# NeuroDiffGym/neurodiffeq

Hardware: NVIDIA H100
Metric: collocation-points/sec (residual+grad) (higher is better)
Workload: dtype f32

## Files before the change

### neurodiffeq_b200/csrc/pinnjet_common.cuh

```cuda
#pragma once
#include <cuda_runtime.h>
#include <stdint.h>
#include <stdlib.h>
#include "pinnjet_plan.h"

namespace pj {

inline bool pdl_enabled() {
    static const int on = [] {
        const char* e = getenv("PINNJET_PDL");
        return (e && e[0] == '1') ? 1 : 0;
    }();
    return on != 0;
}

template <typename... KArgs, typename... Args>
inline cudaError_t launch_kernel(void (*kern)(KArgs...), dim3 grid, dim3 block, size_t smem, cudaStream_t s, bool dependent,
                                 Args&&... args) {
    cudaLaunchConfig_t cfg = {};
    cfg.gridDim = grid;
    cfg.blockDim = block;
    cfg.dynamicSmemBytes = smem;
    cfg.stream = s;
    cudaLaunchAttribute attr[1];
// ... 201 lines not shown

template <int S = 1, typename R>
__device__ __forceinline__ R pg_reduce_scatter8(const R (&v)[8], int pg_lane) {
    const bool b2 = pg_lane & 4, b1 = pg_lane & 2, b0 = pg_lane & 1;
    R w[4], x[2];
#pragma unroll
    for (int i = 0; i < 4; ++i)
        w[i] = (b2 ? v[i + 4] : v[i]) + __shfl_xor_sync(0xffffffffu, b2 ? v[i] : v[i + 4], 4 * S);
#pragma unroll
    for (int i = 0; i < 2; ++i)
        x[i] = (b1 ? w[i + 2] : w[i]) + __shfl_xor_sync(0xffffffffu, b1 ? w[i] : w[i + 2], 2 * S);
    return (b0 ? x[1] : x[0]) + __shfl_xor_sync(0xffffffffu, b0 ? x[0] : x[1], S);
}
template <int S = 1, typename R>
__device__ __forceinline__ R pg_reduce_scatter4(const R (&v)[4], int pg_lane) {
    const bool b2 = pg_lane & 4, b1 = pg_lane & 2;
    R w[2];
#pragma unroll
    for (int i = 0; i < 2; ++i)
        w[i] = (b2 ? v[i + 2] : v[i]) + __shfl_xor_sync(0xffffffffu, b2 ? v[i] : v[i + 2], 4 * S);
    R x = (b1 ? w[1] : w[0]) + __shfl_xor_sync(0xffffffffu, b1 ? w[0] : w[1], 2 * S);
    return x + __shfl_xor_sync(0xffffffffu, x, S);
}

__device__ __forceinline__ float tanh_fast(float x) {
    const float ax = fabsf(x), t = x * x;
    float p = fmaf(-0.006276387721300125f, t, 0.021116213873028755f);
    p = fmaf(p, t, -0.053875137120485306f);
    p = fmaf(p, t, 0.13332924246788025f);
    p = fmaf(p, t, -0.3333333134651184f);
    const float small = fmaf(x * t, p, x);
    float e;
    asm("ex2.approx.ftz.f32 %0, %1;" : "=f"(e) : "f"(fminf(ax, 15.0f) * 2.885390081777927f));
    float r;
    asm("rcp.approx.ftz.f32 %0, %1;" : "=f"(r) : "f"(e + 1.0f));
    const float big = copysignf(fmaf(-2.0f, r, 1.0f), x);
    return ax < 0.6f ? small : big;
}

__device__ __forceinline__ void act_d2(int act, float z0, float& a0, float& s1, float& s2) {
    if (act == PJ_ACT_TANH) {
        a0 = tanh_fast(z0);
        s1 = fmaf(-a0, a0, 1.0f);
        s2 = -2.0f * a0 * s1;
    } else {
        sincosf(z0, &a0, &s1);
// ... 276 lines not shown
#pragma unroll
        for (int q = 0; q < Q; ++q) b[q] = bn[q];
    }
}

__device__ __forceinline__ void split_tf32(float x, uint32_t& big, uint32_t& small) {
    big = (__float_as_uint(x) + 0x1000u) & 0xffffe000u;
    small = __float_as_uint(x - __uint_as_float(big));
}
__device__ __forceinline__ void mma_tf32(float (&d)[4], const uint32_t (&a)[4], const uint32_t (&b)[2]) {
    asm volatile("mma.sync.aligned.m16n8k8.row.col.f32.tf32.tf32.f32 {%0,%1,%2,%3}, {%4,%5,%6,%7}, {%8,%9}, {%0,%1,%2,%3};"
                 : "+f"(d[0]), "+f"(d[1]), "+f"(d[2]), "+f"(d[3])
                 : "r"(a[0]), "r"(a[1]), "r"(a[2]), "r"(a[3]), "r"(b[0]), "r"(b[1]));
}
__device__ __forceinline__ void mma_tf32x3(float (&d)[4], const uint32_t (&ab)[4], const uint32_t (&as)[4], const uint32_t (&bb)[2],
                                           const uint32_t (&bs)[2]) {
    mma_tf32(d, as, bb);
    mma_tf32(d, ab, bs);
    mma_tf32(d, ab, bb);
}

template <typename R, int NTC, int C, int N3>
constexpr bool mma_gemms() { return sizeof(R) == 4 && N3 == 0 && NTC == 128 && C <= 6; }

template <int P, int C, bool AHEAD = true>
__device__ __forceinline__ void gemm_rows_mma(float (&acc)[4][C][P], const float* __restrict__ a_ptr, int RS, int T,
                                              const float* __restrict__ b_ptr, int ldb, int nrows, int lane) {
    static_assert(P == 2 || P == 4, "float2 / float4 point rows");
    const int g = lane >> 2, t = lane & 3;
    const float* ap = a_ptr + 2 * t * RS;
    const float* bp = b_ptr - 4 * t + 4 * (g >> 1) + (g & 1) + 2 * t * ldb;
    struct Ops {
        float a[2][C][P], b[2][2];
    };
    auto load = [&](int k0, Ops& o) {
#pragma unroll
        for (int i = 0; i < 2; ++i) {
            const float* ar = ap + (k0 + i) * RS;
#pragma unroll
            for (int c = 0; c < C; ++c) {
                if constexpr (P == 4) {
                    const float4 v = *reinterpret_cast<const float4*>(ar + c * T);
                    o.a[i][c][0] = v.x;
                    o.a[i][c][1] = v.y;
                    o.a[i][c][2] = v.z;
                    o.a[i][c][3] = v.w;
                } else {
                    const float2 v = *reinterpret_cast<const float2*>(ar + c * T);
                    o.a[i][c][0] = v.x;
                    o.a[i][c][1] = v.y;
                }
            }
#pragma unroll
            for (int ni = 0; ni < 2; ++ni) o.b[ni][i] = bp[(k0 + i) * ldb + 2 * ni];
        }
    };
    if (nrows <= 0) return;
    float d[C][P / 2][2][4];
#pragma unroll
    for (int c = 0; c < C; ++c)
#pragma unroll
        for (int h = 0; h < P / 2; ++h)
#pragma unroll
            for (int ni = 0; ni < 2; ++ni)
#pragma unroll
                for (int e = 0; e < 4; ++e) d[c][h][ni][e] = acc[2 * ni + (e & 1)][c][2 * h + (e >> 1)];
    Ops cur;
    if constexpr (AHEAD) load(0, cur);
#pragma unroll 1
    for (int k0 = 0; k0 < nrows; k0 += 8) {
        Ops nxt;
        if constexpr (AHEAD) load(min(k0 + 8, nrows - 8), nxt);
        else load(k0, cur);
        uint32_t bb[2][2], bs[2][2];
#pragma unroll
        for (int ni = 0; ni < 2; ++ni)
#pragma unroll
            for (int i = 0; i < 2; ++i) split_tf32(cur.b[ni][i], bb[ni][i], bs[ni][i]);
#pragma unroll
        for (int c = 0; c < C; ++c)
#pragma unroll
            for (int h = 0; h < P / 2; ++h) {
                uint32_t ab[4], as[4];
                split_tf32(cur.a[0][c][2 * h], ab[0], as[0]);
                split_tf32(cur.a[0][c][2 * h + 1], ab[1], as[1]);
                split_tf32(cur.a[1][c][2 * h], ab[2], as[2]);
                split_tf32(cur.a[1][c][2 * h + 1], ab[3], as[3]);
#pragma unroll
                for (int ni = 0; ni < 2; ++ni) mma_tf32x3(d[c][h][ni], ab, as, bb[ni], bs[ni]);
            }
        if constexpr (AHEAD) cur = nxt;
    }
#pragma unroll
    for (int c = 0; c < C; ++c)
#pragma unroll
        for (int h = 0; h < P / 2; ++h)
#pragma unroll
            for (int ni = 0; ni < 2; ++ni)
#pragma unroll
                for (int e = 0; e < 4; ++e) acc[2 * ni + (e & 1)][c][2 * h + (e >> 1)] = d[c][h][ni][e];
}

template <typename R, int P, bool SCALAR>
struct GemmAcc {
    typedef typename Pair<R>::type elem;
    static constexpr int n = P / 2;
};
template <int P>
struct GemmAcc<float, P, true> {
    typedef float elem;
    static constexpr int n = P;
};

template <int P, typename PairT>
__device__ __forceinline__ auto pick(const PairT (&v)[P / 2], int p) {
    const auto t = unpack2(v[p >> 1]);
    return (p & 1) ? t.y : t.x;
}
template <int P>
__device__ __forceinline__ float pick(const float (&v)[P], int p) { return v[p]; }

// ... 33 lines not shown
```

### neurodiffeq_b200/csrc/pinnjet_inst.cu

```cuda
#ifndef PJ_WL
#define PJ_WL 0
#endif
#ifndef PJ_N3
#define PJ_N3 0
#endif
#ifndef PJ_XACT
#define PJ_XACT 0
#endif
#define PJ_TC_UNIT (!PJ_F64 && PJ_N3 == 0 && !PJ_XACT)

#include "pinnjet_k1.cuh"
#include "pinnjet_k2.cuh"
#if PJ_TC_UNIT
#include "pinnjet_k1tc3.cuh"
#include "pinnjet_k2tc2.cuh"
#endif

#define PJ_CAT4(a, b, c, d) a##b##_##c##_##d
#define PJ_CAT5(a, b, c, d, e) a##b##_##c##_##d##_##e
#define PJ_NAME4(prefix, n1, n2, wl) PJ_CAT4(prefix, n1, n2, wl)
#define PJ_NAME5(prefix, n1, n2, wl, n3) PJ_CAT5(prefix, n1, n2, wl, n3)
#if PJ_N3 > 0
#define PJ_NAME(prefix, n1, n2) PJ_NAME5(prefix, n1, n2, PJ_WL, PJ_N3)
#else
// ... 39 lines not shown
    const long long i = (long long)blockIdx.x * RED_PARAMS + il;
    red[g][il] = i < n_theta ? red_group_sum(gpart, n_parts, n_theta, i, g) : 0.0f;
    __syncthreads();
    if (g == 0 && i < n_theta) grad[i] += red_combine(red, il);
}

template <typename R>
static cudaError_t launch_reduce_t(const R* gpart, int n_parts, long long n_theta, R* grad, cudaStream_t s) {
    return launch_kernel(k2_reduce_kernel<R>, dim3((unsigned)((n_theta + RED_PARAMS - 1) / RED_PARAMS)), dim3(RED_PARAMS * RED_GROUPS), 0, s,
                         true, gpart, n_parts, n_theta, grad);
}
cudaError_t launch_reduce(const float* gpart, int n_parts, long long n_theta, float* grad, cudaStream_t s) {
    return launch_reduce_t(gpart, n_parts, n_theta, grad, s);
}
cudaError_t launch_reduce_f64(const double* gpart, int n_parts, long long n_theta, double* grad, cudaStream_t s) {
    return launch_reduce_t(gpart, n_parts, n_theta, grad, s);
}

#else

#if PJ_F64
typedef K1ArgsF64 K1A;
typedef K2ArgsF64 K2A;
constexpr int kEsz = 8;
constexpr int kMinB1_128 = 1, kMinB2_128 = 1;
#else
typedef K1Args K1A;
typedef K2Args K2A;
constexpr int kEsz = 4;
constexpr int kMinB1_128 = 3, kMinB2_128 = 2;
#endif
constexpr int kP = ffma_tile_points(1 + PJ_N1 + PJ_N2 + PJ_N3, kEsz);

template <typename Args>
struct Variant {
    void (*kern)(Args);
    int threads;
    cudaError_t ready;
};
template <typename Args>
static Variant<Args> variant(void (*kern)(Args), int threads) {
    return {kern, threads, cudaFuncSetAttribute(kern, cudaFuncAttributeMaxDynamicSharedMemorySize, SMEM_LIMIT)};
}

static Variant<K1A> k1_variant(const Plan& pl) {
#if PJ_TC_UNIT
    if (pl.tc) {
        static const auto v = variant(k1tc3_forward_kernel<PJ_N1, PJ_N2, PJ_WL>, K1T_THREADS);
        return v;
    }
#endif
    if (pl.ntc1 == 128) {
        static const auto v = variant(PJ_K1_KERNEL<128, kMinB1_128, kP, FFMA_Q, PJ_N1, PJ_N2, PJ_WL, PJ_N3>, ffma_k1_threads(128));
        return v;
    }
    if (pl.Q1 == FFMA_Q_WIDE) {
        static const auto v = variant(PJ_K1_KERNEL<256, 1, kP, FFMA_Q_WIDE, PJ_N1, PJ_N2, PJ_WL, PJ_N3>, ffma_k1_threads(256));
        return v;
    }
    static const auto v = variant(PJ_K1_KERNEL<256, 1, kP, FFMA_Q, PJ_N1, PJ_N2, PJ_WL, PJ_N3>, ffma_k1_threads(256));
    return v;
}

static Variant<K2A> k2_variant(const Plan& pl) {
#if PJ_TC_UNIT
    if (pl.tc) {
        static const auto v = variant(k2tc2_backward_kernel<PJ_N1, PJ_N2, PJ_WL>, K2T_THREADS);
        return v;
    }
#endif
    if (pl.n_out_max > K2_OUT_GROUP) {
        if (pl.ntc == 128) {
            static const auto v = variant(PJ_K2_KERNEL<128, kMinB2_128, kP, FFMA_Q, PJ_N1, PJ_N2, PJ_WL, PJ_N3, true>, ffma_k2_threads(128));
            return v;
        }
        static const auto v = variant(PJ_K2_KERNEL<256, 1, kP, FFMA_Q, PJ_N1, PJ_N2, PJ_WL, PJ_N3, true>, ffma_k2_threads(256));
        return v;
    }
    if (pl.ntc == 128) {
        static const auto v = variant(PJ_K2_KERNEL<128, kMinB2_128, kP, FFMA_Q, PJ_N1, PJ_N2, PJ_WL, PJ_N3, false>, ffma_k2_threads(128));
        return v;
    }
    static const auto v = variant(PJ_K2_KERNEL<256, 1, kP, FFMA_Q, PJ_N1, PJ_N2, PJ_WL, PJ_N3, false>, ffma_k2_threads(256));
    return v;
}

template <typename Args>
static cudaError_t launch(const Variant<Args>& v, const Args& a, int grid, int smem, cudaStream_t s) {
    if (v.ready != cudaSuccess) return v.ready;
    return launch_kernel(v.kern, dim3(grid), dim3(v.threads), smem, s, true, a);
}

cudaError_t PJ_NAME(PJ_PREFIX_K1, PJ_N1, PJ_N2)(const K1A& a, int grid, int smem, cudaStream_t s) {
    return launch(k1_variant(a.plan), a, grid, smem, s);
}

cudaError_t PJ_NAME(PJ_PREFIX_K2, PJ_N1, PJ_N2)(const K2A& a, int grid, int smem, cudaStream_t s) {
    return launch(k2_variant(a.plan), a, grid, smem, s);
}

int PJ_NAME(PJ_PREFIX_OCC, PJ_N1, PJ_N2)(const Plan& pl, int k, int smem) {
    int n = 0;
    cudaError_t e;
// ... 14 lines not shown
```

### neurodiffeq_b200/csrc/pinnjet_k2.cuh

```cuda
#pragma once
#include "pinnjet_common.cuh"
#include "pinnjet_k1.cuh"

namespace pj {

constexpr int WJ = 8, WK = 4;

template <typename R>
__device__ __forceinline__ void wgrad_tile(typename Pair<R>::type (&acc)[WJ][WK][1], const R* __restrict__ g_base, int j_step,
                                           const R* __restrict__ z_base, int k_step, int RS, int n_r) {
    typedef typename Pair<R>::row16 row16;
    constexpr int STEP = 16 / sizeof(R);
#pragma unroll 2
    for (int r = 0; r < n_r; r += STEP) {
        row16 gv[WJ], zv[WK];
#pragma unroll
        for (int i = 0; i < WJ; ++i) gv[i] = *reinterpret_cast<const row16*>(g_base + (size_t)i * j_step * RS + r);
#pragma unroll
        for (int i = 0; i < WK; ++i) zv[i] = *reinterpret_cast<const row16*>(z_base + (size_t)i * k_step * RS + r);
#pragma unroll
        for (int i = 0; i < WJ; ++i)
#pragma unroll
            for (int j = 0; j < WK; ++j) Pair<R>::fma16(acc[i][j][0], gv[i], zv[j]);
    }
// ... 5 lines not shown
        float4 gv[WJ], zv[WK];
#pragma unroll
        for (int i = 0; i < WJ; ++i) gv[i] = *reinterpret_cast<const float4*>(g_base + (size_t)i * j_step * RS + r);
#pragma unroll
        for (int i = 0; i < WK; ++i) zv[i] = *reinterpret_cast<const float4*>(z_base + (size_t)i * k_step * RS + r);
#pragma unroll
        for (int i = 0; i < WJ; ++i)
#pragma unroll
            for (int j = 0; j < WK; ++j) {
                acc[i][j][0] = fmaf(gv[i].x, zv[j].x, acc[i][j][0]);
                acc[i][j][1] = fmaf(gv[i].y, zv[j].y, acc[i][j][1]);
                acc[i][j][0] = fmaf(gv[i].z, zv[j].z, acc[i][j][0]);
                acc[i][j][1] = fmaf(gv[i].w, zv[j].w, acc[i][j][1]);
            }
    }
}
template <typename PairT>
__device__ __forceinline__ auto wgrad_sum(const PairT (&v)[1]) {
    const auto t = unpack2(v[0]);
    return t.x + t.y;
}
__device__ __forceinline__ float wgrad_sum(const float (&v)[2]) { return v[0] + v[1]; }

struct WgradMma {
    uint32_t a[2][2][4], b[4][2][2];
    __device__ __forceinline__ void load(const float* __restrict__ g, const float* __restrict__ z, int RS, int r0) {
        const float* gr = g + r0;
        const float* zr = z + r0;
#pragma unroll
        for (int mi = 0; mi < 2; ++mi) {
            const float* p = gr + 16 * mi * RS;
            split_tf32(p[0], a[mi][0][0], a[mi][1][0]);
            split_tf32(p[8 * RS], a[mi][0][1], a[mi][1][1]);
            split_tf32(p[4], a[mi][0][2], a[mi][1][2]);
            split_tf32(p[8 * RS + 4], a[mi][0][3], a[mi][1][3]);
        }
#pragma unroll
        for (int ni = 0; ni < 4; ++ni) {
            const float* p = zr + 8 * ni * RS;
            split_tf32(p[0], b[ni][0][0], b[ni][1][0]);
            split_tf32(p[4], b[ni][0][1], b[ni][1][1]);
        }
    }
};
__device__ __forceinline__ void wgrad_tile_mma(float (&acc)[2][4][4], const float* __restrict__ g_warp,
                                               const float* __restrict__ z_warp, int RS, int n_r, int lane) {
    const int g = lane >> 2, t = lane & 3;
    const float* gb = g_warp + g * RS + t;
    const float* zb = z_warp + g * RS + t;
    WgradMma cur;
    cur.load(gb, zb, RS, 0);
#pragma unroll 1
    for (int r0 = 0; r0 < n_r; r0 += 8) {
        WgradMma nxt;
        nxt.load(gb, zb, RS, min(r0 + 8, n_r - 8));
#pragma unroll
        for (int mi = 0; mi < 2; ++mi)
#pragma unroll
            for (int ni = 0; ni < 4; ++ni) {
                mma_tf32(acc[mi][ni], cur.a[mi][1], cur.b[ni][0]);
                mma_tf32(acc[mi][ni], cur.a[mi][0], cur.b[ni][1]);
                mma_tf32(acc[mi][ni], cur.a[mi][0], cur.b[ni][0]);
            }
        cur = nxt;
    }
}

template <typename R, int NTC, int P, int Q, int N1, int N2, int WL, int N3, bool WIDE, bool XA>
__device__ __forceinline__ void k2_backward_body(const K2ArgsT<R>& A) {
    constexpr int C = 1 + N1 + N2 + N3;
    constexpr bool SCALAR_ACC = sizeof(R) == 4 && N3 == 0;
    constexpr bool MMA = mma_gemms<R, NTC, C, N3>();
    constexpr int PGS = JobMap<MMA>::PG_STEP;
    constexpr int NT_COMPUTE = NTC, NT_TOTAL = NTC + 32, N_CWARPS = NTC / 32;
    extern __shared__ __align__(128) unsigned char smem[];
    const PjSpec& sp = A.spec;
    const Plan& pl = A.plan;
    R* G = reinterpret_cast<R*>(smem + pl.k2_g0);
    R* G2 = reinterpret_cast<R*>(smem + pl.k2_g1);
    R* Zb = reinterpret_cast<R*>(smem + pl.k2_zb);
    R* ring = reinterpret_cast<R*>(smem + pl.k2_ring);
    R* small = reinterpret_cast<R*>(smem + pl.k2_small);
    R* ybar = reinterpret_cast<R*>(smem + pl.k2_ybar);
    R* sgrad = reinterpret_cast<R*>(smem + pl.k2_sgrad);
    uint64_t* full = reinterpret_cast<uint64_t*>(smem + pl.k2_misc);
    uint64_t* empty = full + MAX_STAGES;
    uint64_t* zfull = empty + MAX_STAGES;

    const int tid = threadIdx.x, warp = tid >> 5, lane = tid & 31;
    const int T = pl.T, RS = pl.RS;
    const int my_tiles = (pl.n_tiles > (int)blockIdx.x) ? (pl.n_tiles - 1 - (int)blockIdx.x) / (int)gridDim.x + 1 : 0;
    R* gpart = A.gpart + (size_t)blockIdx.x * sp.n_theta;

    if (tid == 0) {
        for (int s = 0; s < MAX_STAGES; ++s) {
            mbar_init(&full[s], 1);
            mbar_init(&empty[s], N_CWARPS);
        }
        mbar_init(zfull, 1);
        fence_barrier_init();
    }
    pdl_launch_dependents();
    pdl_wait();
    for (int i = tid; i < pl.small_floats; i += NT_TOTAL) small[i] = __ldg(A.pack + i);
    for (int i = tid; i < pl.sgrad_floats * pl.sgrad_copies; i += NT_TOTAL) sgrad[i] = 0.0f;
    for (long long i = tid; i < sp.n_theta; i += NT_TOTAL) gpart[i] = 0.0f;
    __syncthreads();

    if (warp == N_CWARPS) {
        if (lane == 0) weight_producer<false>(sp, A.net, pl, A.pack, ring, full, empty, my_tiles);
        return;
    }

    const JobMap<MMA> jm(tid, T, P, Q);
    const int p0 = jm.p0, u0 = jm.u0;
    R* sg = sgrad + (size_t)(warp % ((T / P) >> 3)) * pl.sgrad_floats;
    RingCursor<R> cur{0, pl.n_stage_bwd, pl.resident_bwd != 0, full, empty, ring};
    uint32_t zphase = 0;
    const int kl = lane & 7, jl = lane >> 3;
    PJ_T_DECL
    PJ_T_MARK(0)

    for (int iter = 0; iter < my_tiles; ++iter) {
        const long long tile = (long long)blockIdx.x + (long long)iter * gridDim.x;
        const long long base = tile * T;
        if (cur.resident) cur.it = 0;
        const R* zj_tile = A.zj + tile * pl.zj_tile_floats;
        const R* seed_tile = A.seeds + tile * ((long long)sp.n_yrows * T);

        for (int n = 0; n < sp.n_nets; ++n) {
            const KNet& net = A.net[n];
            const int L = net.n_linear - 1;
            const int act_kind = net.act;
            const int n_out = net.width[net.n_linear];
            const int hpL = pl.hp[n][L];
            R wq[P][WL > 0 ? WL : 1];
#pragma unroll
            for (int p = 0; p < P; ++p)
#pragma unroll
                for (int dd = 0; dd < (WL > 0 ? WL : 1); ++dd)
                    wq[p][dd] = WL > 0 ? __ldg(A.wts + tile * ((long long)sp.n_nets * WL * T) + (n * WL + dd) * T + p0 + p) : 0.0f;

            if (tid == 0) {
                fence_proxy_async();
                const uint32_t bytes = (uint32_t)(hpL * RS) * (uint32_t)sizeof(R);
                mbar_arrive_expect_tx(zfull, bytes);
                tma_bulk_g2s(Zb, zj_tile + pl.zj_off[n][L], bytes, zfull);
            }
            for (int e = tid; e < n_out * C * T; e += NT_COMPUTE) ybar[e] = __ldg(seed_tile + net.yrow0 * T + e);
            bar_compute<NTC>();
            mbar_wait(zfull, zphase);
            zphase ^= 1u;
            PJ_T_MARK(1)

            {
                const R* wlo = small + pl.s_wlo[n];
                if constexpr (!WIDE) if (u0 < hpL) {
                    static_assert(Q == 4, "the gradient reductions below assume 4 units per thread");
                    static_assert(K2_OUT_GROUP == PJ_MAX_NETS, "the first group's reduction below is written for 4 outputs");
                    R gbq[Q], gwq[K2_OUT_GROUP][Q];
#pragma unroll
                    for (int q = 0; q < Q; ++q) {
                        const int u = u0 + q;
                        R gw[K2_OUT_GROUP];
#pragma unroll
                        for (int o = 0; o < K2_OUT_GROUP; ++o) gw[o] = 0.0f;
                        R gb = 0.0f;
#pragma unroll
                        for (int p = 0; p < P; ++p) {
                            const int pt = p0 + p;
                            R z[C], ab[C], a[C], zb[C];
#pragma unroll
                            for (int c = 0; c < C; ++c) {
                                z[c] = Zb[u * RS + c * T + pt];
                                ab[c] = 0.0f;
                            }
#pragma unroll
                            for (int o = 0; o < K2_OUT_GROUP; ++o)
                                if (o < n_out) {
                                    const R w = wlo[o * hpL + u];
#pragma unroll
                                    for (int c = 0; c < C; ++c) ab[c] = fma(w, ybar[(o * C + c) * T + pt], ab[c]);
                                }
                            act_backward<N1, N2, WL, N3, XA>(act_kind, z, ab, a, zb, wq[p]);
#pragma unroll
                            for (int o = 0; o < K2_OUT_GROUP; ++o)
                                if (o < n_out) {
#pragma unroll
                                    for (int c = 0; c < C; ++c) gw[o] = fma(ybar[(o * C + c) * T + pt], a[c], gw[o]);
                                }
                            gb += zb[0];
#pragma unroll
                            for (int c = 0; c < C; ++c) G[u * RS + c * T + pt] = zb[c];
                        }
                        gbq[q] = gb;
#pragma unroll
                        for (int o = 0; o < K2_OUT_GROUP; ++o) gwq[o][q] = gw[o];
                    }
                    const int pl8 = jm.pg_lane, i4 = pl8 & 3;
                    {
                        const R v0[8] = {gbq[0], gbq[1], gbq[2], gbq[3], gwq[0][0], gwq[0][1], gwq[0][2], gwq[0][3]};
                        const R t0 = pg_reduce_scatter8<PGS>(v0, pl8);
                        if (pl8 < 4) sg[pl.g_b[n][L - 1] + u0 + i4] += t0; else sg[pl.g_wl[n] + u0 + i4] += t0;
                        if (n_out > 1) {
                            const R v1[8] = {gwq[1][0], gwq[1][1], gwq[1][2], gwq[1][3],
                                                 gwq[2][0], gwq[2][1], gwq[2][2], gwq[2][3]};
                            const R t1 = pg_reduce_scatter8<PGS>(v1, pl8);
                            if (pl8 < 4) sg[pl.g_wl[n] + hpL + u0 + i4] += t1;
                            else if (n_out > 2) sg[pl.g_wl[n] + 2 * hpL + u0 + i4] += t1;
                        }
                        if (n_out > 3) {
                            const R v2[4] = {gwq[3][0], gwq[3][1], gwq[3][2], gwq[3][3]};
                            const R t2 = pg_reduce_scatter4<PGS>(v2, pl8);
                            if (!(pl8 & 1)) sg[pl.g_wl[n] + 3 * hpL + u0 + (pl8 >> 1)] += t2;
                        }
                    }
                }
                if constexpr (WIDE) if (u0 < hpL) {
                    R gbq[Q];
#pragma unroll
                    for (int q = 0; q < Q; ++q) {
                        const int u = u0 + q;
                        R gb = 0.0f;
// ... 2 lines not shown
                            const int pt = p0 + p;
                            R z[C], ab[C], a[C], zb[C];
#pragma unroll
                            for (int c = 0; c < C; ++c) {
                                z[c] = Zb[u * RS + c * T + pt];
                                ab[c] = 0.0f;
                            }
                            for (int o = 0; o < n_out; ++o) {
                                const R w = wlo[o * hpL + u];
#pragma unroll
                                for (int c = 0; c < C; ++c) ab[c] = fma(w, ybar[(o * C + c) * T + pt], ab[c]);
                            }
                            act_backward<N1, N2, WL, N3, XA>(act_kind, z, ab, a, zb, wq[p]);
                            gb += zb[0];
#pragma unroll
                            for (int c = 0; c < C; ++c) {
                                G[u * RS + c * T + pt] = zb[c];
                                Zb[u * RS + c * T + pt] = a[c];
                            }
                        }
                        gbq[q] = gb;
                    }
                    const int pl8 = jm.pg_lane, i4 = pl8 & 3;
                    const R tb = pg_reduce_scatter4<PGS>(gbq, pl8);
                    if (!(pl8 & 1)) sg[pl.g_b[n][L - 1] + u0 + (pl8 >> 1)] += tb;
                    for (int o0 = 0; o0 < n_out; o0 += K2_OUT_GROUP) {
                        R gwq[K2_OUT_GROUP][Q];
#pragma unroll
                        for (int q = 0; q < Q; ++q) {
                            const int u = u0 + q;
                            R gw[K2_OUT_GROUP];
#pragma unroll
                            for (int o = 0; o < K2_OUT_GROUP; ++o) gw[o] = 0.0f;
#pragma unroll
                            for (int p = 0; p < P; ++p) {
                                const int pt = p0 + p;
                                R a[C];
#pragma unroll
                                for (int c = 0; c < C; ++c) a[c] = Zb[u * RS + c * T + pt];
#pragma unroll
                                for (int o = 0; o < K2_OUT_GROUP; ++o)
                                    if (o0 + o < n_out) {
#pragma unroll
                                        for (int c = 0; c < C; ++c) gw[o] = fma(ybar[((o0 + o) * C + c) * T + pt], a[c], gw[o]);
                                    }
                            }
#pragma unroll
                            for (int o = 0; o < K2_OUT_GROUP; ++o) gwq[o][q] = gw[o];
                        }
                        const int row = o0 + (pl8 >> 2);
                        const R v1[8] = {gwq[0][0], gwq[0][1], gwq[0][2], gwq[0][3],
                                             gwq[1][0], gwq[1][1], gwq[1][2], gwq[1][3]};
                        const R t1 = pg_reduce_scatter8<PGS>(v1, pl8);
                        if (row < n_out) sg[pl.g_wl[n] + row * hpL + u0 + i4] += t1;
                        if (o0 + 2 < n_out) {
                            const R v2[8] = {gwq[2][0], gwq[2][1], gwq[2][2], gwq[2][3],
                                                 gwq[3][0], gwq[3][1], gwq[3][2], gwq[3][3]};
                            const R t2 = pg_reduce_scatter8<PGS>(v2, pl8);
                            if (row + 2 < n_out) sg[pl.g_wl[n] + (row + 2) * hpL + u0 + i4] += t2;
                        }
                    }
                }
                if (tid < n_out) {
                    R s = 0.0f;
                    for (int pt = 0; pt < T; ++pt) s += ybar[(tid * C) * T + pt];
                    sgrad[pl.g_bout[n] + tid] += s;
                }
            }
            bar_compute<NTC>();
            PJ_T_MARK(2)

            for (int h = L; h >= 2; --h) {
                const int l = h - 1;
                const int HJ = pl.hp[n][h], HK = pl.hp[n][h - 1];
                if (tid == 0) {
                    fence_proxy_async();
                    const uint32_t bytes = (uint32_t)(HK * RS) * (uint32_t)sizeof(R);
                    mbar_arrive_expect_tx(zfull, bytes);
                    tma_bulk_g2s(Zb, zj_tile + pl.zj_off[n][h - 1], bytes, zfull);
                }
                const bool valid = u0 < HK;
                typedef GemmAcc<R, P, SCALAR_ACC> AA;
                typename AA::elem acc[Q][C][AA::n];
#pragma unroll
                for (int q = 0; q < Q; ++q)
#pragma unroll
                    for (int c = 0; c < C; ++c)
#pragma unroll
                        for (int hh = 0; hh < AA::n; ++hh) acc[q][c][hh] = typename AA::elem{};
                const int rpc = chunk_elems(sizeof(R)) / HK;
                for (int r0 = 0; r0 < HJ; r0 += rpc) {
                    const R* chunk = cur.acquire();
                    if (valid) {
                        if constexpr (MMA) gemm_rows_mma<P, C>(acc, G + r0 * RS + p0, RS, T, chunk + u0, HK, min(rpc, HJ - r0), lane);
                        else gemm_rows<P, Q, C>(acc, G + r0 * RS + p0, RS, T, chunk + u0, HK, min(rpc, HJ - r0));
                    }
                    cur.release(lane);
                }
                PJ_T_MARK(3)
                mbar_wait(zfull, zphase);
                zphase ^= 1u;
                PJ_T_MARK(4)
                if (valid) {
                    R gbq[Q];
#pragma unroll
                    for (int q = 0; q < Q; ++q) {
                        const int u = u0 + q;
                        R gb = 0.0f;
                        R av[P][C], zv[P][C];
#pragma unroll
                        for (int p = 0; p < P; ++p) {
                            R z[C], ab[C];
#pragma unroll
                            for (int c = 0; c < C; ++c) {
                                z[c] = Zb[u * RS + c * T + p0 + p];
                                ab[c] = pick<P>(acc[q][c], p);
                            }
                            act_backward<N1, N2, WL, N3, XA>(act_kind, z, ab, av[p], zv[p], wq[p]);
                            gb += zv[p][0];
                        }
#pragma unroll
                        for (int c = 0; c < C; ++c) {
                            if constexpr (P == 4) {
                                store4(Zb + u * RS + c * T + p0, av[0][c], av[1][c], av[2][c], av[3][c]);
                                store4(G2 + u * RS + c * T + p0, zv[0][c], zv[1][c], zv[2][c], zv[3][c]);
                            } else {
                                store2(Zb + u * RS + c * T + p0, av[0][c], av[1][c]);
                                store2(G2 + u * RS + c * T + p0, zv[0][c], zv[1][c]);
                            }
                        }
                        gbq[q] = gb;
                    }
                    const R tb = pg_reduce_scatter4<PGS>(gbq, jm.pg_lane);
                    if (!(jm.pg_lane & 1)) sg[pl.g_b[n][h - 2] + u0 + (jm.pg_lane >> 1)] += tb;
                }
                bar_compute<NTC>();
                PJ_T_MARK(5)
                {
                    const int width_j = net.width[h], width_k = net.width[h - 1];
                    const int n_kb = HK / 32, n_jb = HJ / 32;
                    R* gw = gpart + net.w_off[l];
                    for (int wt = warp; wt < n_kb * n_jb; wt += N_CWARPS) {
                        const int jb = (wt / n_kb) * 32, kb = (wt % n_kb) * 32;
                        if constexpr (MMA) {
                            float wacc[2][4][4] = {};
                            wgrad_tile_mma(wacc, G + (size_t)jb * RS, Zb + (size_t)kb * RS, RS, C * T, lane);
#pragma unroll
                            for (int mi = 0; mi < 2; ++mi)
#pragma unroll
                                for (int ni = 0; ni < 4; ++ni)
#pragma unroll
                                    for (int e = 0; e < 4; ++e) {
                                        const int j = jb + 16 * mi + (lane >> 2) + 8 * (e >> 1);
                                        const int k = kb + 8 * ni + 2 * (lane & 3) + (e & 1);
                                        if (j < width_j && k < width_k) atomicAdd(&gw[(size_t)j * width_k + k], wacc[mi][ni][e]);
                                    }
                        } else {
                            typedef GemmAcc<R, 2, SCALAR_ACC> WA;
                            typename WA::elem wacc[WJ][WK][WA::n];
#pragma unroll
                            for (int i = 0; i < WJ; ++i)
#pragma unroll
                                for (int jj = 0; jj < WK; ++jj)
#pragma unroll
                                    for (int hh = 0; hh < WA::n; ++hh) wacc[i][jj][hh] = typename WA::elem{};
                            wgrad_tile(wacc, G + (size_t)(jb + jl) * RS, 4, Zb + (size_t)(kb + kl) * RS, 8, RS, C * T);
#pragma unroll
                            for (int i = 0; i < WJ; ++i) {
                                const int j = jb + jl + 4 * i;
#pragma unroll
                                for (int jj = 0; jj < WK; ++jj) {
                                    const int k = kb + kl + 8 * jj;
                                    if (j < width_j && k < width_k) atomicAdd(&gw[(size_t)j * width_k + k], wgrad_sum(wacc[i][jj]));
                                }
                            }
                        }
                    }
                }
                bar_compute<NTC>();
                PJ_T_MARK(6)
                R* t = G;
                G = G2;
                G2 = t;
            }

            {
                const int hp1 = pl.hp[n][1];
                if (u0 < hp1) {
                    R x[PJ_MAX_COORDS][P];
#pragma unroll
                    for (int i = 0; i < PJ_MAX_COORDS; ++i)
                        if (i < net.n_in) {
#pragma unroll
                            for (int p = 0; p < P; ++p) {
                                const long long g = min(base + p0 + p, A.N - 1);
                                x[i][p] = __ldg(A.coords[net.in_coord[i]] + g);
                            }
                        }
#pragma unroll
                    for (int q = 0; q < Q; ++q) {
                        const int u = u0 + q;
                        R s0[P];
// ... 10 lines not shown
#pragma unroll
                        for (int i = 0; i < PJ_MAX_COORDS; ++i) {
                            R s = 0.0f;
                            if (i < net.n_in) {
#pragma unroll
                                for (int p = 0; p < P; ++p) s = fma(s0[p], x[i][p], s);
#pragma unroll
                                for (int f = 0; f < N1; ++f) s = fma(sf[f], R(sp.dir[f][net.in_coord[i]]), s);
                            }
                            sv[i] = s;
                        }
                        if (net.n_in <= 4) {
                            const R v4[4] = {sv[0], sv[1], sv[2], sv[3]};
                            const R t = pg_reduce_scatter4<PGS>(v4, jm.pg_lane);
                            const int i = jm.pg_lane >> 1;
                            if (!(jm.pg_lane & 1) && i < net.n_in) sg[pl.g_w0[n] + u * net.n_in + i] += t;
                        } else {
                            const R t = pg_reduce_scatter8<PGS>(sv, jm.pg_lane);
                            if (jm.pg_lane < net.n_in) sg[pl.g_w0[n] + u * net.n_in + jm.pg_lane] += t;
                        }
                    }
                }
            }
            bar_compute<NTC>();
            PJ_T_MARK(7)
        }
    }
    PJ_T_FLUSH(16)

    bar_compute<NTC>();
    for (int n = 0; n < sp.n_nets; ++n) {
        const KNet& net = A.net[n];
        const int L = net.n_linear - 1;
        const int h1 = net.width[1], hL = net.width[L], hpL = pl.hp[n][L], n_out = net.width[net.n_linear];
        auto sgsum = [&](int idx) {
            R v = 0.0f;
            for (int c = 0; c < pl.sgrad_copies; ++c) v += sgrad[(size_t)c * pl.sgrad_floats + idx];
            return v;
        };
        for (int e = tid; e < h1 * net.n_in; e += NT_COMPUTE) gpart[net.w_off[0] + e] += sgsum(pl.g_w0[n] + e);
        for (int hl = 0; hl < L; ++hl)
            for (int e = tid; e < net.width[hl + 1]; e += NT_COMPUTE) gpart[net.b_off[hl] + e] += sgsum(pl.g_b[n][hl] + e);
        for (int e = tid; e < n_out * hL; e += NT_COMPUTE) {
            const int o = e / hL, k = e - o * hL;
            gpart[net.w_off[L] + e] += sgsum(pl.g_wl[n] + o * hpL + k);
        }
        for (int e = tid; e < n_out; e += NT_COMPUTE) gpart[net.b_off[L] + e] += sgsum(pl.g_bout[n] + e);
    }
}

template <int NTC, int MINB, int P, int Q, int N1, int N2, int WL, int N3, bool WIDE>
__global__ void __launch_bounds__(ffma_k2_threads(NTC), MINB) k2_backward_kernel(const __grid_constant__ K2Args A) {
    k2_backward_body<float, NTC, P, Q, N1, N2, WL, N3, WIDE, false>(A);
}
template <int NTC, int MINB, int P, int Q, int N1, int N2, int WL, int N3, bool WIDE>
__global__ void __launch_bounds__(ffma_k2_threads(NTC), MINB) k2_backward_kernel_f64(const __grid_constant__ K2ArgsF64 A) {
    k2_backward_body<double, NTC, P, Q, N1, N2, WL, N3, WIDE, false>(A);
}
template <int NTC, int MINB, int P, int Q, int N1, int N2, int WL, int N3, bool WIDE>
__global__ void __launch_bounds__(ffma_k2_threads(NTC), MINB) k2_backward_kernel_xact(const __grid_constant__ K2Args A) {
    k2_backward_body<float, NTC, P, Q, N1, N2, WL, N3, WIDE, true>(A);
}
template <int NTC, int MINB, int P, int Q, int N1, int N2, int WL, int N3, bool WIDE>
__global__ void __launch_bounds__(ffma_k2_threads(NTC), MINB) k2_backward_kernel_f64_xact(const __grid_constant__ K2ArgsF64 A) {
    k2_backward_body<double, NTC, P, Q, N1, N2, WL, N3, WIDE, true>(A);
}

}
```

### neurodiffeq_b200/csrc/pinnjet_plan.h

```cpp
#pragma once
#include "../../include/pinnjet.h"

namespace pj {

constexpr int SMEM_LIMIT = 232448;
constexpr int SMEM_PER_SM = 233472;

constexpr int CHUNK_BYTES = 16384;
constexpr int CHUNK_FLOATS = CHUNK_BYTES / 4;
constexpr int chunk_elems(int esz) { return CHUNK_BYTES / esz; }
constexpr int MAX_STAGES = 8;
constexpr int ROW_PAD = 4;
constexpr int row_pad(int esz) { return 16 / esz; }
constexpr int ffma_tile_points(int C, int esz = 4) { return C <= 2 && esz == 4 ? 4 : 2; }
constexpr int FFMA_Q = 4, FFMA_Q_WIDE = 8;
constexpr int K2_OUT_GROUP = 4;
constexpr int ffma_k1_threads(int ntc) { return ntc + (ntc == 128 ? 32 : 64); }
constexpr int ffma_k2_threads(int ntc) { return ntc + 32; }

constexpr int TC_ROWS = 128;
constexpr int TC_H = 64;
constexpr int TC_AIMG = TC_ROWS * 128;
constexpr int TC_WIMG = TC_H * 128;
constexpr int TC_WOUT = 16 * 128;
constexpr int TC_NCW = 16;
constexpr int TC_NT = TC_NCW * 32;
constexpr int TC_STAGE_STRIDE = 20;
constexpr int TC_STAGE_BYTES = TC_NCW * 32 * TC_STAGE_STRIDE * 4;
constexpr int tc_channel_pad(int C) { return C <= 2 ? 2 : (C <= 4 ? 4 : 8); }
constexpr int K1T_NPW = 2;
constexpr int K1T_THREADS = TC_NT + 32 + 32 * K1T_NPW + 32;
constexpr int K1T_EB = 32 * K1T_NPW;
constexpr int K1T_RING = 4;
constexpr int K2T_THREADS = TC_NT + 64;
constexpr int TC_PROG_RESERVE = 8192;

constexpr int PROG_MAX = 2048;
constexpr int SLOTS_MAX = 128;

constexpr int LOSS_PART_BYTES = 4096;
constexpr int LOSS_TICKET_WORD = 639;
// ... 73 lines not shown
```

Measured before the change: 81.65 million.

## Double compute warps in MMA backward kernel and drop dedicated weight producer warp

For the tensor-core (MMA) path of the backward kernel, the block now runs 2*NTC compute threads, each handling half as many hidden units (Q=2), instead of NTC compute threads plus a producer warp. Weight chunks are issued by thread 0 after each barrier, replacing the producer warp and empty-barrier handshake, with each whole hidden matrix loaded as one chunk. Reductions, GEMM and weight-gradient tiling get Q=2 variants. This aims at more warps to hide MMA and shuffle latency, at the cost of more threads per block, register pressure against the minimum-blocks bound, and less overlap of weight loads.

```diff
diff --git a/neurodiffeq_b200/csrc/pinnjet_common.cuh b/neurodiffeq_b200/csrc/pinnjet_common.cuh
--- a/neurodiffeq_b200/csrc/pinnjet_common.cuh
+++ b/neurodiffeq_b200/csrc/pinnjet_common.cuh
@@ -247,6 +247,13 @@
     R x = (b1 ? w[1] : w[0]) + __shfl_xor_sync(0xffffffffu, b1 ? w[0] : w[1], 2 * S);
     return x + __shfl_xor_sync(0xffffffffu, x, S);
 }
+template <int S = 1, typename R>
+__device__ __forceinline__ R pg_reduce_scatter2(const R (&v)[2], int pg_lane) {
+    const bool b2 = pg_lane & 4;
+    R x = (b2 ? v[1] : v[0]) + __shfl_xor_sync(0xffffffffu, b2 ? v[0] : v[1], 4 * S);
+    x += __shfl_xor_sync(0xffffffffu, x, 2 * S);
+    return x + __shfl_xor_sync(0xffffffffu, x, S);
+}
 
 __device__ __forceinline__ float tanh_fast(float x) {
     const float ax = fabsf(x), t = x * x;
@@ -569,16 +576,20 @@
 
 template <typename R, int NTC, int C, int N3>
 constexpr bool mma_gemms() { return sizeof(R) == 4 && N3 == 0 && NTC == 128 && C <= 6; }
-
-template <int P, int C, bool AHEAD = true>
-__device__ __forceinline__ void gemm_rows_mma(float (&acc)[4][C][P], const float* __restrict__ a_ptr, int RS, int T,
+template <typename R, int NTC, int C, int N3>
+constexpr int k2_block_threads() { return ffma_k2_threads(NTC, mma_gemms<R, NTC, C, N3>()); }
+
+template <int P, int C, bool AHEAD = true, int Q = 4>
+__device__ __forceinline__ void gemm_rows_mma(float (&acc)[Q][C][P], const float* __restrict__ a_ptr, int RS, int T,
                                               const float* __restrict__ b_ptr, int ldb, int nrows, int lane) {
     static_assert(P == 2 || P == 4, "float2 / float4 point rows");
+    static_assert(Q == 2 || Q == 4, "one or two n8 tiles");
+    constexpr int NI = Q / 2;
     const int g = lane >> 2, t = lane & 3;
     const float* ap = a_ptr + 2 * t * RS;
-    const float* bp = b_ptr - 4 * t + 4 * (g >> 1) + (g & 1) + 2 * t * ldb;
+    const float* bp = Q == 4 ? b_ptr - 4 * t + 4 * (g >> 1) + (g & 1) + 2 * t * ldb : b_ptr - 2 * t + g + 2 * t * ldb;
     struct Ops {
-        float a[2][C][P], b[2][2];
+        float a[2][C][P], b[NI][2];
     };
     auto load = [&](int k0, Ops& o) {
 #pragma unroll
@@ -599,17 +610,17 @@
                 }
             }
 #pragma unroll
-            for (int ni = 0; ni < 2; ++ni) o.b[ni][i] = bp[(k0 + i) * ldb + 2 * ni];
+            for (int ni = 0; ni < NI; ++ni) o.b[ni][i] = bp[(k0 + i) * ldb + 2 * ni];
         }
     };
     if (nrows <= 0) return;
-    float d[C][P / 2][2][4];
+    float d[C][P / 2][NI][4];
 #pragma unroll
     for (int c = 0; c < C; ++c)
 #pragma unroll
         for (int h = 0; h < P / 2; ++h)
 #pragma unroll
-            for (int ni = 0; ni < 2; ++ni)
+            for (int ni = 0; ni < NI; ++ni)
 #pragma unroll
                 for (int e = 0; e < 4; ++e) d[c][h][ni][e] = acc[2 * ni + (e & 1)][c][2 * h + (e >> 1)];
     Ops cur;
@@ -619,9 +630,9 @@
         Ops nxt;
         if constexpr (AHEAD) load(min(k0 + 8, nrows - 8), nxt);
         else load(k0, cur);
-        uint32_t bb[2][2], bs[2][2];
-#pragma unroll
-        for (int ni = 0; ni < 2; ++ni)
+        uint32_t bb[NI][2], bs[NI][2];
+#pragma unroll
+        for (int ni = 0; ni < NI; ++ni)
 #pragma unroll
             for (int i = 0; i < 2; ++i) split_tf32(cur.b[ni][i], bb[ni][i], bs[ni][i]);
 #pragma unroll
@@ -634,7 +645,7 @@
                 split_tf32(cur.a[1][c][2 * h], ab[2], as[2]);
                 split_tf32(cur.a[1][c][2 * h + 1], ab[3], as[3]);
 #pragma unroll
-                for (int ni = 0; ni < 2; ++ni) mma_tf32x3(d[c][h][ni], ab, as, bb[ni], bs[ni]);
+                for (int ni = 0; ni < NI; ++ni) mma_tf32x3(d[c][h][ni], ab, as, bb[ni], bs[ni]);
             }
         if constexpr (AHEAD) cur = nxt;
     }
@@ -643,7 +654,7 @@
 #pragma unroll
         for (int h = 0; h < P / 2; ++h)
 #pragma unroll
-            for (int ni = 0; ni < 2; ++ni)
+            for (int ni = 0; ni < NI; ++ni)
 #pragma unroll
                 for (int e = 0; e < 4; ++e) acc[2 * ni + (e & 1)][c][2 * h + (e >> 1)] = d[c][h][ni][e];
 }
diff --git a/neurodiffeq_b200/csrc/pinnjet_inst.cu b/neurodiffeq_b200/csrc/pinnjet_inst.cu
--- a/neurodiffeq_b200/csrc/pinnjet_inst.cu
+++ b/neurodiffeq_b200/csrc/pinnjet_inst.cu
@@ -85,15 +85,18 @@
 #if PJ_F64
 typedef K1ArgsF64 K1A;
 typedef K2ArgsF64 K2A;
+typedef double KR;
 constexpr int kEsz = 8;
 constexpr int kMinB1_128 = 1, kMinB2_128 = 1;
 #else
 typedef K1Args K1A;
 typedef K2Args K2A;
+typedef float KR;
 constexpr int kEsz = 4;
 constexpr int kMinB1_128 = 3, kMinB2_128 = 2;
 #endif
 constexpr int kP = ffma_tile_points(1 + PJ_N1 + PJ_N2 + PJ_N3, kEsz);
+constexpr int kK2Threads128 = k2_block_threads<KR, 128, 1 + PJ_N1 + PJ_N2 + PJ_N3, PJ_N3>();
 
 template <typename Args>
 struct Variant {
@@ -134,14 +137,14 @@
 #endif
     if (pl.n_out_max > K2_OUT_GROUP) {
         if (pl.ntc == 128) {
-            static const auto v = variant(PJ_K2_KERNEL<128, kMinB2_128, kP, FFMA_Q, PJ_N1, PJ_N2, PJ_WL, PJ_N3, true>, ffma_k2_threads(128));
+            static const auto v = variant(PJ_K2_KERNEL<128, kMinB2_128, kP, FFMA_Q, PJ_N1, PJ_N2, PJ_WL, PJ_N3, true>, kK2Threads128);
             return v;
         }
         static const auto v = variant(PJ_K2_KERNEL<256, 1, kP, FFMA_Q, PJ_N1, PJ_N2, PJ_WL, PJ_N3, true>, ffma_k2_threads(256));
         return v;
     }
     if (pl.ntc == 128) {
-        static const auto v = variant(PJ_K2_KERNEL<128, kMinB2_128, kP, FFMA_Q, PJ_N1, PJ_N2, PJ_WL, PJ_N3, false>, ffma_k2_threads(128));
+        static const auto v = variant(PJ_K2_KERNEL<128, kMinB2_128, kP, FFMA_Q, PJ_N1, PJ_N2, PJ_WL, PJ_N3, false>, kK2Threads128);
         return v;
     }
     static const auto v = variant(PJ_K2_KERNEL<256, 1, kP, FFMA_Q, PJ_N1, PJ_N2, PJ_WL, PJ_N3, false>, ffma_k2_threads(256));
diff --git a/neurodiffeq_b200/csrc/pinnjet_k2.cuh b/neurodiffeq_b200/csrc/pinnjet_k2.cuh
--- a/neurodiffeq_b200/csrc/pinnjet_k2.cuh
+++ b/neurodiffeq_b200/csrc/pinnjet_k2.cuh
@@ -51,8 +51,9 @@
 }
 __device__ __forceinline__ float wgrad_sum(const float (&v)[2]) { return v[0] + v[1]; }
 
+template <int NI>
 struct WgradMma {
-    uint32_t a[2][2][4], b[4][2][2];
+    uint32_t a[2][2][4], b[NI][2][2];
     __device__ __forceinline__ void load(const float* __restrict__ g, const float* __restrict__ z, int RS, int r0) {
         const float* gr = g + r0;
         const float* zr = z + r0;
@@ -65,28 +66,29 @@
             split_tf32(p[8 * RS + 4], a[mi][0][3], a[mi][1][3]);
         }
 #pragma unroll
-        for (int ni = 0; ni < 4; ++ni) {
+        for (int ni = 0; ni < NI; ++ni) {
             const float* p = zr + 8 * ni * RS;
             split_tf32(p[0], b[ni][0][0], b[ni][1][0]);
             split_tf32(p[4], b[ni][0][1], b[ni][1][1]);
         }
     }
 };
-__device__ __forceinline__ void wgrad_tile_mma(float (&acc)[2][4][4], const float* __restrict__ g_warp,
+template <int NI>
+__device__ __forceinline__ void wgrad_tile_mma(float (&acc)[2][NI][4], const float* __restrict__ g_warp,
                                                const float* __restrict__ z_warp, int RS, int n_r, int lane) {
     const int g = lane >> 2, t = lane & 3;
     const float* gb = g_warp + g * RS + t;
     const float* zb = z_warp + g * RS + t;
-    WgradMma cur;
+    WgradMma<NI> cur;
     cur.load(gb, zb, RS, 0);
 #pragma unroll 1
     for (int r0 = 0; r0 < n_r; r0 += 8) {
-        WgradMma nxt;
+        WgradMma<NI> nxt;
         nxt.load(gb, zb, RS, min(r0 + 8, n_r - 8));
 #pragma unroll
         for (int mi = 0; mi < 2; ++mi)
 #pragma unroll
-            for (int ni = 0; ni < 4; ++ni) {
+            for (int ni = 0; ni < NI; ++ni) {
                 mma_tf32(acc[mi][ni], cur.a[mi][1], cur.b[ni][0]);
                 mma_tf32(acc[mi][ni], cur.a[mi][0], cur.b[ni][1]);
                 mma_tf32(acc[mi][ni], cur.a[mi][0], cur.b[ni][0]);
@@ -95,13 +97,35 @@
     }
 }
 
-template <typename R, int NTC, int P, int Q, int N1, int N2, int WL, int N3, bool WIDE, bool XA>
+template <typename R>
+__device__ __forceinline__ void feed_weight_chunk(const PjSpec& sp, const KNet* nets, const Plan& pl, const R* __restrict__ pack,
+                                                  R* ring, uint64_t* full, int i) {
+    int j = i % pl.chunks_bwd;
+    for (int n = 0; n < sp.n_nets; ++n) {
+        const int nm = nets[n].n_linear - 2;
+        if (j < nm) {
+            const int l = nm - j;
+            const int stage = i % pl.n_stage_bwd;
+            const uint32_t bytes = (uint32_t)(pl.hp[n][l + 1] * pl.hp[n][l]) * (uint32_t)sizeof(R);
+            mbar_arrive_expect_tx(&full[stage], bytes);
+            tma_bulk_g2s(ring + (size_t)stage * chunk_elems(sizeof(R)), pack + pl.b_wo[n][l], bytes, &full[stage]);
+            return;
+        }
+        j -= nm;
+    }
+}
+
+template <typename R, int NTC, int P, int QP, int N1, int N2, int WL, int N3, bool WIDE, bool XA>
 __device__ __forceinline__ void k2_backward_body(const K2ArgsT<R>& A) {
     constexpr int C = 1 + N1 + N2 + N3;
     constexpr bool SCALAR_ACC = sizeof(R) == 4 && N3 == 0;
     constexpr bool MMA = mma_gemms<R, NTC, C, N3>();
     constexpr int PGS = JobMap<MMA>::PG_STEP;
-    constexpr int NT_COMPUTE = NTC, NT_TOTAL = NTC + 32, N_CWARPS = NTC / 32;
+    constexpr int Q = MMA ? QP / 2 : QP;
+    constexpr int NT_COMPUTE = MMA ? 2 * NTC : NTC, NT_TOTAL = ffma_k2_threads(NTC, MMA), N_CWARPS = NT_COMPUTE / 32;
+    static_assert(!MMA || (QP == 4 && 64 * 64 * sizeof(R) <= CHUNK_BYTES),
+                  "the weight feed takes every hidden->hidden matrix (at most 64 x 64 for 128-thread plans) as one chunk, so "
+                  "one adjoint GEMM never waits on a chunk that only its own barrier would free");
     extern __shared__ __align__(128) unsigned char smem[];
     const PjSpec& sp = A.spec;
     const Plan& pl = A.plan;
@@ -124,7 +148,7 @@
     if (tid == 0) {
         for (int s = 0; s < MAX_STAGES; ++s) {
             mbar_init(&full[s], 1);
-            mbar_init(&empty[s], N_CWARPS);
+            if constexpr (!MMA) mbar_init(&empty[s], N_CWARPS);
         }
         mbar_init(zfull, 1);
         fence_barrier_init();
@@ -136,7 +160,11 @@
     for (long long i = tid; i < sp.n_theta; i += NT_TOTAL) gpart[i] = 0.0f;
     __syncthreads();
 
-    if (warp == N_CWARPS) {
+    const int feed_total = my_tiles > 0 ? (pl.resident_bwd ? pl.chunks_bwd : my_tiles * pl.chunks_bwd) : 0;
+    if constexpr (MMA) {
+        if (tid == 0)
+            for (int i = 0; i < min(pl.n_stage_bwd, feed_total); ++i) feed_weight_chunk(sp, A.net, pl, A.pack, ring, full, i);
+    } else if (warp == N_CWARPS) {
         if (lane == 0) weight_producer<false>(sp, A.net, pl, A.pack, ring, full, empty, my_tiles);
         return;
     }
@@ -177,7 +205,7 @@
                 tma_bulk_g2s(Zb, zj_tile + pl.zj_off[n][L], bytes, zfull);
             }
             for (int e = tid; e < n_out * C * T; e += NT_COMPUTE) ybar[e] = __ldg(seed_tile + net.yrow0 * T + e);
-            bar_compute<NTC>();
+            bar_compute<NT_COMPUTE>();
             mbar_wait(zfull, zphase);
             zphase ^= 1u;
             PJ_T_MARK(1)
@@ -185,7 +213,6 @@
             {
                 const R* wlo = small + pl.s_wlo[n];
                 if constexpr (!WIDE) if (u0 < hpL) {
-                    static_assert(Q == 4, "the gradient reductions below assume 4 units per thread");
                     static_assert(K2_OUT_GROUP == PJ_MAX_NETS, "the first group's reduction below is written for 4 outputs");
                     R gbq[Q], gwq[K2_OUT_GROUP][Q];
 #pragma unroll
@@ -227,7 +254,19 @@
                         for (int o = 0; o < K2_OUT_GROUP; ++o) gwq[o][q] = gw[o];
                     }
                     const int pl8 = jm.pg_lane, i4 = pl8 & 3;
-                    {
+                    if constexpr (Q == 2) {
+                        const R v0[8] = {gbq[0], gbq[1], gwq[0][0], gwq[0][1], gwq[1][0], gwq[1][1], gwq[2][0], gwq[2][1]};
+                        const R t0 = pg_reduce_scatter8<PGS>(v0, pl8);
+                        const int row = (pl8 >> 1) - 1, u = u0 + (pl8 & 1);
+                        if (row < 0) sg[pl.g_b[n][L - 1] + u] += t0;
+                        else if (row < n_out) sg[pl.g_wl[n] + row * hpL + u] += t0;
+                        if (n_out > 3) {
+                            const R v2[2] = {gwq[3][0], gwq[3][1]};
+                            const R t2 = pg_reduce_scatter2<PGS>(v2, pl8);
+                            if (!(pl8 & 3)) sg[pl.g_wl[n] + 3 * hpL + u0 + (pl8 >> 2)] += t2;
+                        }
+                    } else {
+                        static_assert(Q == 4, "the gradient reductions below assume 4 units per thread");
                         const R v0[8] = {gbq[0], gbq[1], gbq[2], gbq[3], gwq[0][0], gwq[0][1], gwq[0][2], gwq[0][3]};
                         const R t0 = pg_reduce_scatter8<PGS>(v0, pl8);
                         if (pl8 < 4) sg[pl.g_b[n][L - 1] + u0 + i4] += t0; else sg[pl.g_wl[n] + u0 + i4] += t0;
@@ -276,8 +315,13 @@
                         gbq[q] = gb;
                     }
                     const int pl8 = jm.pg_lane, i4 = pl8 & 3;
-                    const R tb = pg_reduce_scatter4<PGS>(gbq, pl8);
-                    if (!(pl8 & 1)) sg[pl.g_b[n][L - 1] + u0 + (pl8 >> 1)] += tb;
+                    if constexpr (Q == 2) {
+                        const R tb = pg_reduce_scatter2<PGS>(gbq, pl8);
+                        if (!(pl8 & 3)) sg[pl.g_b[n][L - 1] + u0 + (pl8 >> 2)] += tb;
+                    } else {
+                        const R tb = pg_reduce_scatter4<PGS>(gbq, pl8);
+                        if (!(pl8 & 1)) sg[pl.g_b[n][L - 1] + u0 + (pl8 >> 1)] += tb;
+                    }
                     for (int o0 = 0; o0 < n_out; o0 += K2_OUT_GROUP) {
                         R gwq[K2_OUT_GROUP][Q];
 #pragma unroll
@@ -302,16 +346,23 @@
 #pragma unroll
                             for (int o = 0; o < K2_OUT_GROUP; ++o) gwq[o][q] = gw[o];
                         }
-                        const int row = o0 + (pl8 >> 2);
-                        const R v1[8] = {gwq[0][0], gwq[0][1], gwq[0][2], gwq[0][3],
-                                             gwq[1][0], gwq[1][1], gwq[1][2], gwq[1][3]};
-                        const R t1 = pg_reduce_scatter8<PGS>(v1, pl8);
-                        if (row < n_out) sg[pl.g_wl[n] + row * hpL + u0 + i4] += t1;
-                        if (o0 + 2 < n_out) {
-                            const R v2[8] = {gwq[2][0], gwq[2][1], gwq[2][2], gwq[2][3],
-                                                 gwq[3][0], gwq[3][1], gwq[3][2], gwq[3][3]};
-                            const R t2 = pg_reduce_scatter8<PGS>(v2, pl8);
-                            if (row + 2 < n_out) sg[pl.g_wl[n] + (row + 2) * hpL + u0 + i4] += t2;
+                        if constexpr (Q == 2) {
+                            const int row = o0 + (pl8 >> 1);
+                            const R v1[8] = {gwq[0][0], gwq[0][1], gwq[1][0], gwq[1][1], gwq[2][0], gwq[2][1], gwq[3][0], gwq[3][1]};
+                            const R t1 = pg_reduce_scatter8<PGS>(v1, pl8);
+                            if (row < n_out) sg[pl.g_wl[n] + row * hpL + u0 + (pl8 & 1)] += t1;
+                        } else {
+                            const int row = o0 + (pl8 >> 2);
+                            const R v1[8] = {gwq[0][0], gwq[0][1], gwq[0][2], gwq[0][3],
+                                                 gwq[1][0], gwq[1][1], gwq[1][2], gwq[1][3]};
+                            const R t1 = pg_reduce_scatter8<PGS>(v1, pl8);
+                            if (row < n_out) sg[pl.g_wl[n] + row * hpL + u0 + i4] += t1;
+                            if (o0 + 2 < n_out) {
+                                const R v2[8] = {gwq[2][0], gwq[2][1], gwq[2][2], gwq[2][3],
+                                                     gwq[3][0], gwq[3][1], gwq[3][2], gwq[3][3]};
+                                const R t2 = pg_reduce_scatter8<PGS>(v2, pl8);
+                                if (row + 2 < n_out) sg[pl.g_wl[n] + (row + 2) * hpL + u0 + i4] += t2;
+                            }
                         }
                     }
                 }
@@ -321,7 +372,7 @@
                     sgrad[pl.g_bout[n] + tid] += s;
                 }
             }
-            bar_compute<NTC>();
+            bar_compute<NT_COMPUTE>();
             PJ_T_MARK(2)
 
             for (int h = L; h >= 2; --h) {
@@ -342,14 +393,17 @@
                     for (int c = 0; c < C; ++c)
 #pragma unroll
                         for (int hh = 0; hh < AA::n; ++hh) acc[q][c][hh] = typename AA::elem{};
-                const int rpc = chunk_elems(sizeof(R)) / HK;
-                for (int r0 = 0; r0 < HJ; r0 += rpc) {
+                if constexpr (MMA) {
                     const R* chunk = cur.acquire();
-                    if (valid) {
-                        if constexpr (MMA) gemm_rows_mma<P, C>(acc, G + r0 * RS + p0, RS, T, chunk + u0, HK, min(rpc, HJ - r0), lane);
-                        else gemm_rows<P, Q, C>(acc, G + r0 * RS + p0, RS, T, chunk + u0, HK, min(rpc, HJ - r0));
-                    }
-                    cur.release(lane);
+                    if (valid) gemm_rows_mma<P, C, true, Q>(acc, G + p0, RS, T, chunk + u0, HK, HJ, lane);
+                    ++cur.it;
+                } else {
+                    const int rpc = chunk_elems(sizeof(R)) / HK;
+                    for (int r0 = 0; r0 < HJ; r0 += rpc) {
+                        const R* chunk = cur.acquire();
+                        if (valid) gemm_rows<P, Q, C>(acc, G + r0 * RS + p0, RS, T, chunk + u0, HK, min(rpc, HJ - r0));
+                        cur.release(lane);
+                    }
                 }
                 PJ_T_MARK(3)
                 mbar_wait(zfull, zphase);
@@ -385,24 +439,35 @@
                         }
                         gbq[q] = gb;
                     }
-                    const R tb = pg_reduce_scatter4<PGS>(gbq, jm.pg_lane);
-                    if (!(jm.pg_lane & 1)) sg[pl.g_b[n][h - 2] + u0 + (jm.pg_lane >> 1)] += tb;
-                }
-                bar_compute<NTC>();
+                    if constexpr (Q == 2) {
+                        const R tb = pg_reduce_scatter2<PGS>(gbq, jm.pg_lane);
+                        if (!(jm.pg_lane & 3)) sg[pl.g_b[n][h - 2] + u0 + (jm.pg_lane >> 2)] += tb;
+                    } else {
+                        const R tb = pg_reduce_scatter4<PGS>(gbq, jm.pg_lane);
+                        if (!(jm.pg_lane & 1)) sg[pl.g_b[n][h - 2] + u0 + (jm.pg_lane >> 1)] += tb;
+                    }
+                }
+                bar_compute<NT_COMPUTE>();
+                if constexpr (MMA)
+                    if (tid == 0 && !cur.resident && cur.it - 1 + pl.n_stage_bwd < feed_total) {
+                        fence_proxy_async();
+                        feed_weight_chunk(sp, A.net, pl, A.pack, ring, full, cur.it - 1 + pl.n_stage_bwd);
+                    }
                 PJ_T_MARK(5)
                 {
                     const int width_j = net.width[h], width_k = net.width[h - 1];
-                    const int n_kb = HK / 32, n_jb = HJ / 32;
+                    constexpr int WTK = MMA ? 8 * Q : 32;
+                    const int n_kb = HK / WTK, n_jb = HJ / 32;
                     R* gw = gpart + net.w_off[l];
                     for (int wt = warp; wt < n_kb * n_jb; wt += N_CWARPS) {
-                        const int jb = (wt / n_kb) * 32, kb = (wt % n_kb) * 32;
+                        const int jb = (wt / n_kb) * 32, kb = (wt % n_kb) * WTK;
                         if constexpr (MMA) {
-                            float wacc[2][4][4] = {};
+                            float wacc[2][WTK / 8][4] = {};
                             wgrad_tile_mma(wacc, G + (size_t)jb * RS, Zb + (size_t)kb * RS, RS, C * T, lane);
 #pragma unroll
                             for (int mi = 0; mi < 2; ++mi)
 #pragma unroll
-                                for (int ni = 0; ni < 4; ++ni)
+                                for (int ni = 0; ni < WTK / 8; ++ni)
 #pragma unroll
                                     for (int e = 0; e < 4; ++e) {
                                         const int j = jb + 16 * mi + (lane >> 2) + 8 * (e >> 1);
@@ -431,7 +496,7 @@
                         }
                     }
                 }
-                bar_compute<NTC>();
+                bar_compute<NT_COMPUTE>();
                 PJ_T_MARK(6)
                 R* t = G;
                 G = G2;
@@ -488,13 +553,13 @@
                     }
                 }
             }
-            bar_compute<NTC>();
+            bar_compute<NT_COMPUTE>();
             PJ_T_MARK(7)
         }
     }
     PJ_T_FLUSH(16)
 
-    bar_compute<NTC>();
+    bar_compute<NT_COMPUTE>();
     for (int n = 0; n < sp.n_nets; ++n) {
         const KNet& net = A.net[n];
         const int L = net.n_linear - 1;
@@ -516,7 +581,7 @@
 }
 
 template <int NTC, int MINB, int P, int Q, int N1, int N2, int WL, int N3, bool WIDE>
-__global__ void __launch_bounds__(ffma_k2_threads(NTC), MINB) k2_backward_kernel(const __grid_constant__ K2Args A) {
+__global__ void __launch_bounds__((k2_block_threads<float, NTC, 1 + N1 + N2 + N3, N3>()), MINB) k2_backward_kernel(const __grid_constant__ K2Args A) {
     k2_backward_body<float, NTC, P, Q, N1, N2, WL, N3, WIDE, false>(A);
 }
 template <int NTC, int MINB, int P, int Q, int N1, int N2, int WL, int N3, bool WIDE>
@@ -524,7 +589,7 @@
     k2_backward_body<double, NTC, P, Q, N1, N2, WL, N3, WIDE, false>(A);
 }
 template <int NTC, int MINB, int P, int Q, int N1, int N2, int WL, int N3, bool WIDE>
-__global__ void __launch_bounds__(ffma_k2_threads(NTC), MINB) k2_backward_kernel_xact(const __grid_constant__ K2Args A) {
+__global__ void __launch_bounds__((k2_block_threads<float, NTC, 1 + N1 + N2 + N3, N3>()), MINB) k2_backward_kernel_xact(const __grid_constant__ K2Args A) {
     k2_backward_body<float, NTC, P, Q, N1, N2, WL, N3, WIDE, true>(A);
 }
 template <int NTC, int MINB, int P, int Q, int N1, int N2, int WL, int N3, bool WIDE>
diff --git a/neurodiffeq_b200/csrc/pinnjet_plan.h b/neurodiffeq_b200/csrc/pinnjet_plan.h
--- a/neurodiffeq_b200/csrc/pinnjet_plan.h
+++ b/neurodiffeq_b200/csrc/pinnjet_plan.h
@@ -16,7 +16,7 @@
 constexpr int FFMA_Q = 4, FFMA_Q_WIDE = 8;
 constexpr int K2_OUT_GROUP = 4;
 constexpr int ffma_k1_threads(int ntc) { return ntc + (ntc == 128 ? 32 : 64); }
-constexpr int ffma_k2_threads(int ntc) { return ntc + 32; }
+constexpr int ffma_k2_threads(int ntc, bool eight_warps = false) { return eight_warps ? 2 * ntc : ntc + 32; }
 
 constexpr int TC_ROWS = 128;
 constexpr int TC_H = 64;
```

Result: faster. 86.62 million, median of 6 (+6.1%).
